# huahbo/IBAMR

Measured on AMD Instinct MI355X. Metric: IB_4 3D spread+interp marker-ops/sec (fp64) + % HBM roofline, 1/2/4/8 GPU, higher is better.
Workload: dtype f64; 1 GPU; cfg4: 1024^3 periodic staggered grid, 1e8 uniform markers (seed 1234), IB_4, z-slabs; kernel=IB_4, markers=100000000, parallelism=z-slab x1, marker_order=cell, layout=packed, spread_mode=one rank, move=False, renumber=False, spread_into=zeroed f (LDataManager::spread, LDataManager.cpp:596), overlap=False

## Files before the change

### ibamr_amd/csrc/le_sweep.hip

```cpp
#include <hip/hip_runtime.h>

#include <climits>
#include <type_traits>
#include <cstdio>
#include <cstdlib>

#include "le_internal.h"
#include "le_stencil.h"

namespace ibtk_le {

constexpr int SW = 64;
#ifndef IBTK_LE_DIAG_SPREAD
#define IBTK_LE_DIAG_SPREAD 0
#endif

__device__ __forceinline__ double lds_ld(const double* q) {
    return *(const volatile __attribute__((address_space(3))) double*)q;
}

__device__ __forceinline__ int lane_id() { return __lane_id(); }

struct D3 {
    double v[3];
// ... 617 lines not shown
        const double Xraw = (FAM == 2) ? p.X[(int64_t)3 * s + d] : Xs[d];
        stencil1d<K>(Xs[d], Xraw, cd.xlo[d], p.bg.dx[d], cd.ilower[d], cd.lo[d], cd.hi[d], d == cd.axis, p.K6, st[d]);
    }
    const int ox = st[0].icl - gx0, oy = st[1].icl - gy0, oz = st[2].icl - zorg;
    bool ok;
    if constexpr (FAM == 0) {
        ok = ox >= 0 && ox + W <= RX - cd.xcell && oy >= 0 && oy + W <= S::RY - cd.ycell && oz >= a + S::LO &&
             oz + W - 1 <= a + S::HI;
    } else {
        bool empty = false;
#pragma unroll
        for (int d = 0; d < 3; ++d) empty = empty || st[d].ist > st[d].isp;
        if (empty) return 0.0;
        ok = ox + st[0].ist >= 0 && ox + st[0].isp < RX && oy + st[1].ist >= 0 && oy + st[1].isp < S::RY &&
             oz + st[2].ist >= a + S::LO && oz + st[2].isp <= a + S::HI;
    }
    if (!ok) {
        atomicOr(p.err, 1);
        return 0.0;
    }
    double acc = 0.0;
    if constexpr (FAM == 3) {
        acc = ring[islot<K>(oz) * PV + oy * RX + ox];
    } else if constexpr (FAM == 0) {
        const double* base = ring + oy * RX + ox;
        constexpr int R = W <= 4 ? W : (W <= 6 ? 3 : 2);
#pragma unroll
        for (int i2 = 0; i2 < W; ++i2) {
            const double* pl = base + islot<K>(oz + i2) * PV;
#pragma unroll
            for (int r0 = 0; r0 < W; r0 += R) {
                double v[R * W];
#pragma unroll
                for (int r = 0; r < R; ++r)
#pragma unroll
                    for (int i0 = 0; i0 < W; ++i0)
                        v[r * W + i0] = lds_ld(&pl[(r0 + r) * RX + i0]);
#pragma unroll
                for (int r = 0; r < R; ++r) {
                    const double wyz = st[1].w[r0 + r] * st[2].w[i2];
#pragma unroll
                    for (int i0 = 0; i0 < W; ++i0) {
                        const double wt = st[0].w[i0] * wyz;
                        acc = acc + wt * v[r * W + i0];
                    }
                }
            }
        }

    } else {
        double w[3][W];
        int o[3][W];
#pragma unroll
        for (int d = 0; d < 3; ++d) {
#pragma unroll
            for (int i = 0; i < W; ++i) {
                const bool in = i >= st[d].ist && i <= st[d].isp;
                w[d][i] = in ? st[d].w[i] : 0.0;
                o[d][i] = min(max(i, st[d].ist), st[d].isp);
            }
        }
#pragma unroll
        for (int i2 = 0; i2 < W; ++i2) {
            const double* pl = ring + islot<K>(oz + o[2][i2]) * PV + oy * RX + ox;
#pragma unroll
            for (int i1 = 0; i1 < W; ++i1) {
#pragma unroll
                for (int i0 = 0; i0 < W; ++i0)
                    acc = acc + w[0][i0] * w[1][i1] * w[2][i2] * pl[o[1][i1] * RX + o[0][i0]];
            }
        }
    }
    return acc;
}

constexpr int LVL_REC = 32;
__device__ __forceinline__ unsigned lvl_class(const int2* tab, int dx, int dy, int dz, int n0, int n1, int n2,
                                              int64_t s1, int64_t s2) {
    const int2 e = tab[dx + 3 * dy + 9 * dz];
    const int64_t shift = e.y ? (int64_t)dx * n0 + (int64_t)dy * n1 * s1 + (int64_t)dz * n2 * s2 : 0;
    return (unsigned)e.x - (unsigned)(8 * shift);
}
template <int K, bool LVL, bool LF = false>
__global__ __launch_bounds__(SW * IWAVES) void k_interp_sweep(Params p) {
    static_assert(LVL || !LF, "the fused fill is a level's");
    using S = ISh<K>;
    constexpr int LO = S::LO, HI = S::HI, RX = S::RX, NPT = S::NPT;
    __shared__ double ring[S::NSL * S::PVP];
    const int it = sweep_item(p, p.ncomp);
    if (it < 0) return;
    int c;
    SweepItem si;
    item_decode(p, it, c, si);
    const int col = si.col;
    const int a0 = si.p0, a1 = si.p1;
    const int lane = lane_id();
    const int w = __builtin_amdgcn_readfirstlane((int)threadIdx.x >> 6);
    ColGeom cg;
    CompDesc cd;
    const int* bs;
    item_patch<LVL>(p, si, c, cg, cd, bs);
    gdouble* const sorted_X = cur_sorted_X(p);
    if (p.zmode) {
        const bool inner = cg.org[2] + a0 + LO >= p.zlo && cg.org[2] + a1 - 1 + HI <= p.zhi;
        if (inner != (p.zmode == 1)) return;
    }
    {
        bool any = false;
        for (int a = a0 + lane; a < a1; a += SW) any = any || bs[bucket(cg, a, col, NBAND)] > bs[bucket(cg, a, col, 0)];
        if (!__any(any)) return;
    }
    const int cx = col % cg.ncx, cy = col / cg.ncx;
    const int gx0 = cg.org[0] + cx * COLX + LO, gy0 = cg.org[1] + cy * COLY + LO;
    const int zorg = cg.org[2];
    const int nlast = p.nsorted - 1;
    auto image = [&](int i, int d) {
        if (!p.iper[d] || (i >= cd.ilower[d] && i <= cd.iupper[d])) return i;
        const int n = cd.iupper[d] - cd.ilower[d] + 1;
        int r = (i - cd.ilower[d]) % n;
        return cd.ilower[d] + (r < 0 ? r + n : r);
    };
    const bool xlast = S::FAM == 0 && cd.xcell, ylast = S::FAM == 0 && cd.ycell;
    unsigned poff[NPT];
#pragma unroll
    for (int k = 0; k < NPT; ++k) {
        const int q = min(lane + SW * k, S::PV - 1);
        const int qx = q % RX, qy = q / RX;
        const int gx = gx0 + qx, gy = gy0 + qy;
        const bool in = gx >= cd.lo[0] && gx <= cd.hi[0] && gy >= cd.lo[1] && gy <= cd.hi[1] &&
                        !(xlast && qx == RX - 1) && !(ylast && qy == S::RY - 1);
        poff[k] = in ? 8u * (unsigned)((image(gx, 0) - cd.lo[0]) + (image(gy, 1) - cd.lo[1]) * (int)cd.s1) : OFF_NONE;
    }
    constexpr bool lfill = LF;
    unsigned lsel = 0;
    struct Cls {
        unsigned o0, o1, o2, o3;
    };
    Cls ob_m{}, ob_0{}, ob_p{};
    const double* lbase = nullptr;
    unsigned lspan = 0;
    int sxd = 0, syd = 0;
    if constexpr (LF) {
        {
            sxd = gx0 < cd.ilower[0] ? -1 : (gx0 + RX - 1 >= cd.ilower[0] + p.lvl_n[0] ? 1 : 0);
            syd = gy0 < cd.ilower[1] ? -1 : (gy0 + S::RY - 1 >= cd.ilower[1] + p.lvl_n[1] ? 1 : 0);
            const int2* rec = p.lvl_nbr + ((int64_t)c * p.npatch + si.patch) * LVL_REC;
            const int2* tab = rec + 13;
            const int n0 = p.lvl_n[0], n1 = p.lvl_n[1], n2 = p.lvl_n[2];
            const int64_t s1 = cd.s1, s2 = cd.s2;
            ob_m = Cls{lvl_class(tab, 0, 0, -1, n0, n1, n2, s1, s2), lvl_class(tab, sxd, 0, -1, n0, n1, n2, s1, s2),
                       lvl_class(tab, 0, syd, -1, n0, n1, n2, s1, s2), lvl_class(tab, sxd, syd, -1, n0, n1, n2, s1, s2)};
            ob_0 = Cls{lvl_class(tab, 0, 0, 0, n0, n1, n2, s1, s2), lvl_class(tab, sxd, 0, 0, n0, n1, n2, s1, s2),
                       lvl_class(tab, 0, syd, 0, n0, n1, n2, s1, s2), lvl_class(tab, sxd, syd, 0, n0, n1, n2, s1, s2)};
            ob_p = Cls{lvl_class(tab, 0, 0, 1, n0, n1, n2, s1, s2), lvl_class(tab, sxd, 0, 1, n0, n1, n2, s1, s2),
                       lvl_class(tab, 0, syd, 1, n0, n1, n2, s1, s2), lvl_class(tab, sxd, syd, 1, n0, n1, n2, s1, s2)};
            const int2 wb = rec[27], ws = rec[28];
            lbase = reinterpret_cast<const double*>(((uint64_t)(unsigned)wb.y << 32) | (unsigned)wb.x);
            lspan = (unsigned)ws.x;
#pragma unroll
            for (int k = 0; k < NPT; ++k) {
                const int q = min(lane + SW * k, S::PV - 1);
                const int gx = gx0 + q % RX, gy = gy0 + q / RX;
                const bool bx = gx < cd.ilower[0] || gx >= cd.ilower[0] + p.lvl_n[0];
                const bool by = gy < cd.ilower[1] || gy >= cd.ilower[1] + p.lvl_n[1];
                lsel |= ((bx ? 1u : 0u) | (by ? 2u : 0u)) << (2 * k);
            }
        }
    }
    const int plast = a1 - 1 + HI;
    const unsigned plane_bytes = (unsigned)(8 * cd.s2);
    auto plane_load = [&](int zr, double* v) __attribute__((always_inline)) {
        const int z0 = zorg + min(zr, plast);
        const bool zin = z0 >= cd.lo[2] && z0 <= cd.hi[2];
        if constexpr (LF) {
            {
                const int dz = z0 < cd.ilower[2] ? -1 : (z0 >= cd.ilower[2] + p.lvl_n[2] ? 1 : 0);
                const unsigned zo = (unsigned)(8 * (int64_t)(z0 - cd.lo[2]) * cd.s2);
                const unsigned mm = 0u - (unsigned)(dz < 0), mp = 0u - (unsigned)(dz > 0), m0 = ~(mm | mp);
                const unsigned O0 = ((ob_m.o0 & mm) | (ob_0.o0 & m0) | (ob_p.o0 & mp)) + zo;
                const unsigned O1 = ((ob_m.o1 & mm) | (ob_0.o1 & m0) | (ob_p.o1 & mp)) + zo;
                const unsigned O2 = ((ob_m.o2 & mm) | (ob_0.o2 & m0) | (ob_p.o2 & mp)) + zo;
                const unsigned O3 = ((ob_m.o3 & mm) | (ob_0.o3 & m0) | (ob_p.o3 & mp)) + zo;
                const auto pb = plane_rsrc(lbase, zin ? lspan : 0u);
#pragma unroll
                for (int k = 0; k < NPT; ++k) {
                    const unsigned cl = (lsel >> (2 * k)) & 3u;
                    const unsigned o = (cl & 2u) ? ((cl & 1u) ? O3 : O2) : ((cl & 1u) ? O1 : O0);
                    v[k] = buf_ld(pb, poff[k] == OFF_NONE ? OFF_NONE : poff[k] + o);
                }
                return;
            }
        }
        const int z = zin ? image(z0, 2) : z0;
        const int zc = min(max(z, cd.lo[2]), cd.hi[2]);
        const auto pb = plane_rsrc(cd.u + (int64_t)(zc - cd.lo[2]) * cd.s2, zin ? plane_bytes : 0u);
#pragma unroll
        for (int k = 0; k < NPT; ++k) v[k] = buf_ld(pb, poff[k]);
    };
    auto plane_put = [&](int zr, const double* v) {
        double* sl = ring + islot<K>(zr) * S::PVP;
#pragma unroll
        for (int k = 0; k < NPT; ++k)
            if (S::PV % SW == 0 || k < NPT - 1 || lane + SW * k < S::PV) sl[lane + SW * k] = v[k];
    };
    struct Mk {
        int s;
        int q;
        double X[3];
    };
    auto lds_barrier = [&]() {
        asm volatile("s_waitcnt lgkmcnt(0)" ::: "memory");
        __builtin_amdgcn_s_barrier();
        asm volatile("" ::: "memory");
    };

    struct GSpan {
        int beg[IWAVES];
        int pre[IWAVES + 1];
    };
    auto gspan_load = [&](int a) {
        const int k = lane < IWAVES ? lane : min(lane - IWAVES, IWAVES - 1);
        const int ac = min(a + k, cg.nz - 1);
        return bs[bucket(cg, ac, col, lane >= IWAVES && lane < 2 * IWAVES ? NBAND : 0)];
    };
    auto gspan_get = [&](int a, int v, GSpan& gsp) {
        int acc = 0;
#pragma unroll
        for (int k = 0; k < IWAVES; ++k) {
            const int b = __builtin_amdgcn_readlane(v, k);
            const int e = a + k < a1 ? __builtin_amdgcn_readlane(v, IWAVES + k) : b;
            gsp.beg[k] = b;
            gsp.pre[k] = acc;
            acc += e - b;
        }
        gsp.pre[IWAVES] = acc;
    };
    auto chunk_load = [&](const GSpan& gsp, int a, int c, Mk& m, int& am) {
        const int tot = gsp.pre[IWAVES];
        const int j = min(SW * c + lane, max(tot - 1, 0));
        int e = gsp.beg[0] + j, k = 0;
#pragma unroll
        for (int q = 1; q < IWAVES; ++q)
            if (j >= gsp.pre[q]) {
                e = gsp.beg[q] + (j - gsp.pre[q]);
                k = q;
            }
        am = a + k;
        e = min(e, nlast);
        m.s = p.sorted_s[e];
        m.q = (p.qdst ? p.qdst : p.sorted_s)[e];
        const D3 xs = ld3(sorted_X + (int64_t)3 * e);
        m.X[0] = xs.v[0];
        m.X[1] = xs.v[1];
        m.X[2] = xs.v[2];
    };
    auto process_pool = [&](int n, const Mk& m, int am) {
        const bool act = lane < n;
        double acc = 0.0;
        if (act) acc = interp_marker<K>(p, cd, ring, gx0, gy0, zorg, am, m.X, m.s);
        double* dst = (act && m.q >= 0) ? p.Qout + ((int64_t)p.Q_depth * m.q + cd.qcomp) : p.sink + lane;
        *dst = acc;
    };
    double pv[NPT];
    for (int z = a0 + LO + w; z < a0 + HI; z += IWAVES) {
        plane_load(z, pv);
        plane_put(z, pv);
    }
    plane_load(a0 + w + HI, pv);
    GSpan gs;
    gspan_get(a0, gspan_load(a0), gs);
    Mk nxt;
    int anx;
    chunk_load(gs, a0, w, nxt, anx);
    int vsp1 = gspan_load(a0 + IWAVES);
    for (int a = a0; a < a1; a += IWAVES) {
        const int my = a + w;
        lds_barrier();
        plane_put(my + HI, pv);
        lds_barrier();
        const Mk cur = nxt;
        const int acur = anx;
        const GSpan gc = gs;

        gspan_get(a + IWAVES, vsp1, gs);
        chunk_load(gs, a + IWAVES, w, nxt, anx);
        vsp1 = gspan_load(a + 2 * IWAVES);
        plane_load(my + IWAVES + HI, pv);
        const int tot = gc.pre[IWAVES];
        if (SW * w < tot) {
            Mk m = cur;
            int am = acur;
            for (int c = w; SW * c < tot; c += IWAVES) {
                const Mk now = m;
                const int anow = am;
                if (SW * (c + IWAVES) < tot) chunk_load(gc, a, c + IWAVES, m, am);
                process_pool(min(tot - SW * c, SW), now, anow);
            }
        }
    }
}

constexpr int I3C = 3;
constexpr int I3PAD = 11;
constexpr int I3WPC = 4, I3PF = 1;
template <int K> struct I3Sh {
    using S = ISh<K>;
    static constexpr int RSTR = S::NSL * S::PVP + I3PAD;
    static constexpr size_t lds = sizeof(double) * I3C * RSTR;
    static constexpr bool fits = S::FAM == 0 && lds <= 160 * 1024;
};
template <int K, int WPC, int PF>
__global__ __launch_bounds__(SW * I3C * WPC) void k_interp3(Params p) {
    using S = ISh<K>;
    static_assert(I3Sh<K>::fits, "k_interp3: closed-form kernels whose three rings fit the LDS");
    static_assert(IWAVES % WPC == 0, "a component's new planes of a group split evenly over its waves");
    constexpr int LO = S::LO, HI = S::HI, RX = S::RX, NPT = S::NPT, PVP = S::PVP;
    constexpr int PPW = IWAVES / WPC;
    constexpr int I3M = WPC * SW;
    constexpr int RSTR = I3Sh<K>::RSTR;
    __shared__ double ring[I3C * RSTR];
    const int it = sweep_item(p, 1);
    if (it < 0) return;
    const SweepItem si = p.items[it];
    const int col = si.col;
    const int a0 = si.p0, a1 = si.p1;
    const int lane = lane_id();
    const int w = __builtin_amdgcn_readfirstlane((int)threadIdx.x >> 6);
    const int cw = w / WPC, jw = w - cw * WPC;
    const ColGeom& cg = p.cg;
    const int* const bs = p.plane_start;
    gdouble* const sorted_X = cur_sorted_X(p);
    if (p.zmode) {
        const bool inner = cg.org[2] + a0 + LO >= p.zlo && cg.org[2] + a1 - 1 + HI <= p.zhi;
        if (inner != (p.zmode == 1)) return;
    }
    {
        bool any = false;
        for (int a = a0 + lane; a < a1; a += SW) any = any || bs[bucket(cg, a, col, NBAND)] > bs[bucket(cg, a, col, 0)];
        if (!__any(any)) return;
    }
    const int cx = col % cg.ncx, cy = col / cg.ncx;
    const int gx0 = cg.org[0] + cx * COLX + LO, gy0 = cg.org[1] + cy * COLY + LO;
    const int zorg = cg.org[2];
    const int nlast = p.nsorted - 1;
    const CompDesc cd = cw == 0 ? p.comp[0] : (cw == 1 ? p.comp[1] : p.comp[2]);
    auto image = [&](int i, int d) {
        if (!p.iper[d] || (i >= cd.ilower[d] && i <= cd.iupper[d])) return i;
        const int n = cd.iupper[d] - cd.ilower[d] + 1;
        int r = (i - cd.ilower[d]) % n;
        return cd.ilower[d] + (r < 0 ? r + n : r);
    };
    const bool xlast = cd.xcell, ylast = cd.ycell;
    unsigned poff[NPT];
#pragma unroll
    for (int k = 0; k < NPT; ++k) {
        const int q = min(lane + SW * k, S::PV - 1);
        const int qx = q % RX, qy = q / RX;
        const int gx = gx0 + qx, gy = gy0 + qy;
        const bool in = gx >= cd.lo[0] && gx <= cd.hi[0] && gy >= cd.lo[1] && gy <= cd.hi[1] &&
                        !(xlast && qx == RX - 1) && !(ylast && qy == S::RY - 1);
        poff[k] = in ? 8u * (unsigned)((image(gx, 0) - cd.lo[0]) + (image(gy, 1) - cd.lo[1]) * (int)cd.s1) : OFF_NONE;
    }
    const int plast = a1 - 1 + HI;
    const unsigned plane_bytes = (unsigned)(8 * cd.s2);
    auto plane_load = [&](int zr, double* v) __attribute__((always_inline)) {
        const int z0 = zorg + min(zr, plast);
        const bool zin = z0 >= cd.lo[2] && z0 <= cd.hi[2];
        const int z = zin ? image(z0, 2) : z0;
        const int zc = min(max(z, cd.lo[2]), cd.hi[2]);
        const auto pb = plane_rsrc(cd.u + (int64_t)(zc - cd.lo[2]) * cd.s2, zin ? plane_bytes : 0u);
#pragma unroll
        for (int k = 0; k < NPT; ++k) v[k] = buf_ld(pb, poff[k]);
    };
    double* const ring_w = ring + cw * RSTR;
    auto plane_put = [&](int zr, const double* v) {
        double* sl = ring_w + islot<K>(zr) * PVP;
#pragma unroll
        for (int k = 0; k < NPT; ++k)
            if (S::PV % SW == 0 || k < NPT - 1 || lane + SW * k < S::PV) sl[lane + SW * k] = v[k];
    };
    const int cl = (int)threadIdx.x % I3C, ml = (int)threadIdx.x / I3C;
    CompDesc cdl;
#define I3SEL(f) cdl.f = cl == 0 ? p.comp[0].f : (cl == 1 ? p.comp[1].f : p.comp[2].f)
#pragma unroll
    for (int d = 0; d < 3; ++d) {
        I3SEL(xlo[d]);
        I3SEL(ilower[d]);
        I3SEL(lo[d]);
        I3SEL(hi[d]);
    }
    I3SEL(axis);
    I3SEL(xcell);
    I3SEL(ycell);
    I3SEL(qcomp);
#undef I3SEL
    const double* const ring_l = ring + cl * RSTR;
    struct Mk {
        int q;
        double X[3];
    };
    auto lds_barrier = [&]() {
        asm volatile("s_waitcnt lgkmcnt(0)" ::: "memory");
        __builtin_amdgcn_s_barrier();
        asm volatile("" ::: "memory");
    };
    struct GSpan {
        int beg[IWAVES];
        int pre[IWAVES + 1];
    };
    auto gspan_load = [&](int a) {
        const int k = lane < IWAVES ? lane : min(lane - IWAVES, IWAVES - 1);
        const int ac = min(a + k, cg.nz - 1);
        return bs[bucket(cg, ac, col, lane >= IWAVES && lane < 2 * IWAVES ? NBAND : 0)];
    };
    auto gspan_get = [&](int a, int v, GSpan& gsp) {
        int acc = 0;
#pragma unroll
        for (int k = 0; k < IWAVES; ++k) {
            const int b = __builtin_amdgcn_readlane(v, k);
            const int e = a + k < a1 ? __builtin_amdgcn_readlane(v, IWAVES + k) : b;
            gsp.beg[k] = b;
            gsp.pre[k] = acc;
            acc += e - b;
        }
        gsp.pre[IWAVES] = acc;
    };
    auto mk_load = [&](const GSpan& gsp, int a, int r, Mk& m, int& am) {
        const int tot = gsp.pre[IWAVES];
        const int j = min(I3M * r + ml, max(tot - 1, 0));
        int e = gsp.beg[0] + j, k = 0;
#pragma unroll
        for (int q = 1; q < IWAVES; ++q)
            if (j >= gsp.pre[q]) {
                e = gsp.beg[q] + (j - gsp.pre[q]);
                k = q;
            }
        am = a + k;
        e = min(e, nlast);
        m.q = (p.qdst ? p.qdst : p.sorted_s)[e];
        const D3 xs = ld3(sorted_X + (int64_t)3 * e);
        m.X[0] = xs.v[0];
        m.X[1] = xs.v[1];
        m.X[2] = xs.v[2];
    };
    auto process = [&](int n, const Mk& m, int am) {
        const bool act = ml < n;
        double acc = 0.0;
        if (act) acc = interp_marker<K>(p, cdl, ring_l, gx0, gy0, zorg, am, m.X, 0);
        double* dst = (act && m.q >= 0) ? p.Qout + ((int64_t)p.Q_depth * m.q + cdl.qcomp) : p.sink + lane;
        *dst = acc;
    };
    {
        double pv[NPT];
        for (int z = a0 + LO + jw; z < a0 + HI; z += WPC) {
            plane_load(z, pv);
            plane_put(z, pv);
        }
    }
    double pv[PF][PPW][NPT];
#pragma unroll
    for (int b = 0; b < PF; ++b)
#pragma unroll
        for (int t = 0; t < PPW; ++t) plane_load(a0 + b * IWAVES + jw + WPC * t + HI, pv[b][t]);
    GSpan gs;
    gspan_get(a0, gspan_load(a0), gs);
    Mk nxt;
    int anx;
    mk_load(gs, a0, 0, nxt, anx);
    int vsp1 = gspan_load(a0 + IWAVES);
    auto group = [&](int a, double (*pvb)[NPT]) __attribute__((always_inline)) {
        lds_barrier();
#pragma unroll
        for (int t = 0; t < PPW; ++t) plane_put(a + jw + WPC * t + HI, pvb[t]);
        lds_barrier();
        const Mk cur = nxt;
        const int acur = anx;
        const GSpan gc = gs;
        gspan_get(a + IWAVES, vsp1, gs);
        mk_load(gs, a + IWAVES, 0, nxt, anx);
        vsp1 = gspan_load(a + 2 * IWAVES);
#pragma unroll
        for (int t = 0; t < PPW; ++t) plane_load(a + PF * IWAVES + jw + WPC * t + HI, pvb[t]);
        const int tot = gc.pre[IWAVES];
        Mk m = cur;
        int am = acur;
        for (int r = 0; I3M * r < tot; ++r) {
            const Mk now = m;
            const int anow = am;
            if (I3M * (r + 1) < tot) mk_load(gc, a, r + 1, m, am);
            process(min(tot - I3M * r, I3M), now, anow);
        }
    };
    for (int a = a0; a < a1; a += PF * IWAVES) {
#pragma unroll
        for (int b = 0; b < PF; ++b)
            if (b == 0 || a + b * IWAVES < a1) group(a + b * IWAVES, pv[b]);
    }
}

__global__ __launch_bounds__(BLOCK) void k_interp_outside_col(Params p, int n) {
    const int first = p.plane_start[p.nbuckets_total];
    for (int e = first + blockIdx.x * BLOCK + threadIdx.x; e < n; e += gridDim.x * BLOCK) {
        const int s = p.qdst ? p.qdst[e] : p.sorted_s[e];
        if (s < 0) continue;
        for (int c = 0; c < p.ncomp; ++c) p.Qout[(int64_t)p.Q_depth * s + p.comp[c].qcomp] = 0.0;
    }
}

template <int K, bool ZC = false> struct SSh {
    using T = KT<K>;
    static constexpr int W = T::W, LO = T::LO, HI = T::HI, FAM = T::FAM;
    static_assert(!ZC || FAM == 0, "the key-frame ring: closed-form kernels");
    static constexpr int HIE = ZC ? HI - 1 : HI;
    static constexpr int NS = HIE - LO + 1;
    static constexpr int NSL = NS + 1;
    static constexpr int PV = COLX * COLY;
    static constexpr int NPL = PV / SW;
    static constexpr int NR = 11;
    static_assert(NS <= 16, "plane field");
    static_assert(COLX == 32 && COLY % 4 == 0 && COLY >= 8, "32-point rows of 4 x 4 tiles; bands need COLY >= 8");
};

__device__ __forceinline__ void ring_xy(int i, int& x, int& y) {
    const int t = i >> 4, j = i & 15;
    x = 4 * (t % (COLX / 4)) + (j & 3);
    y = 4 * (t / (COLX / 4)) + (j >> 2);
}
__device__ __forceinline__ int ring_wrapped(int x, int y) {
    const int xw = x & (COLX - 1);
    const int yw = ((y % COLY) + COLY) % COLY;
    return 16 * ((xw >> 2) + (COLX / 4) * (yw >> 2)) + (xw & 3) + 4 * (yw & 3);
}

template <class S> __device__ __forceinline__ int sslot(int prel) {
    return (int)((unsigned)(prel + 16 * S::NSL) % (unsigned)S::NSL);
}

struct Ranges {
    int start[SSh<K_IB_4>::NR];
    int pre[SSh<K_IB_4>::NR + 1];
};
__device__ __forceinline__ void make_ranges_lanes(const int* rowv, Ranges& R) {
    constexpr int NR = SSh<K_IB_4>::NR;
    constexpr int rr[NR] = {0, 0, 0, 0, 0, 1, 2, 2, 2, 2, 2};
    constexpr int ib[NR] = {8, 11, 14, 17, 20, 6, 6, 9, 12, 15, 18};
    constexpr int ie[NR] = {9, 12, 15, 18, 21, 21, 7, 10, 13, 16, 19};
    int acc = 0;
#pragma unroll
    for (int r = 0; r < NR; ++r) {
        const int b = __builtin_amdgcn_readlane(rowv[rr[r]], ib[r]);
        const int e = __builtin_amdgcn_readlane(rowv[rr[r]], ie[r]);
        R.start[r] = b;
        R.pre[r] = acc;
        acc += e - b;
    }
    R.pre[NR] = acc;
}
__device__ __forceinline__ int range_pos(const Ranges& R, int j) {
    constexpr int NR = SSh<K_IB_4>::NR;
    int pos = R.start[0] + j;
#pragma unroll
    for (int r = 1; r < NR; ++r)
        if (j >= R.pre[r]) pos = R.start[r] + (j - R.pre[r]);
    return pos;
}

constexpr int CS_PTAB = 2048;
__device__ __forceinline__ bool ca_decode(const Params& p, int ca, ColGeom& cg, int& col, int& a, const int*& bs,
                                          int& zb, double& zxlo, int& zilo, const int* ptab) {
    int base = 0;
    if (p.pd) {
        int lo = 0, hi = p.npatch - 1;
        while (lo < hi) {
            const int mid = (lo + hi + 1) >> 1;
            if ((ptab ? ptab[mid] : p.pd[mid].bucket_base / NBAND) <= ca) lo = mid;
            else hi = mid - 1;
        }
        const PatchDesc& P = p.pd[lo];
        cg = P.cg;
        base = P.bucket_base / NBAND;
        bs = p.plane_start + P.bucket_base;
        zb = P.ca_base_z;
        zxlo = P.xlo[2] - 0.5 * p.bg.dx[2];
        zilo = P.ilower[2];
    } else {
        cg = p.cg;
        bs = p.plane_start;
        zb = 0;
        zxlo = p.bg.xlo[2] - 0.5 * p.bg.dx[2];
        zilo = p.bg.ilower[2];
    }
    const int l = ca - base;
    col = l / cg.nz;
    a = l - col * cg.nz;
    zb += col * (cg.nz + 1) + a;
    const int cx = col % cg.ncx, cy = col / cg.ncx;
    return !(cx == 0 || cx == cg.ncx - 1 || cy == 0 || cy == cg.ncy - 1);
}
__device__ __forceinline__ void ca_range(const ColGeom& cg, const int* bs, int col, int a, int r, int& b, int& e) {
    constexpr int rr[11] = {0, 0, 0, 0, 0, 1, 2, 2, 2, 2, 2};
    constexpr int ib[11] = {8, 11, 14, 17, 20, 6, 6, 9, 12, 15, 18};
    constexpr int ie[11] = {9, 12, 15, 18, 21, 21, 7, 10, 13, 16, 19};
    const int cx = col % cg.ncx, cy = col / cg.ncx;
    const int base = bucket(cg, a, (cy - 1 + rr[r]) * cg.ncx + (cx - 1), 0);
    b = bs[base + ib[r]];
    e = bs[base + ie[r]];
}
constexpr int CS_GRID = 8192;
__device__ __forceinline__ bool cs_stands(const Params& p) {
    return p.items_skip && *p.items_skip == 0 && (!p.cs_off_z || *p.cs_zflip != p.cs_epoch);
}
__device__ __forceinline__ const int* cs_patch_table(const Params& p, int* ptab) {
    if (!p.pd || p.npatch > CS_PTAB) return nullptr;
    for (int q = threadIdx.x; q < p.npatch; q += BLOCK) ptab[q] = p.pd[q].bucket_base / NBAND;
    __syncthreads();
    return ptab;
}
__global__ __launch_bounds__(BLOCK) void k_cand_count(Params p, int ncl, int* cnt) {
    if (cs_stands(p)) return;
    __shared__ int ptab_s[CS_PTAB];
    const int* const ptab = cs_patch_table(p, ptab_s);
    for (int ca = blockIdx.x * BLOCK + threadIdx.x; ca < ncl; ca += gridDim.x * BLOCK) {
        ColGeom cg;
        int col, a, zb, zilo;
        double zxlo;
        const int* bs;
        int t = 0;
        if (ca_decode(p, ca, cg, col, a, bs, zb, zxlo, zilo, ptab)) {
#pragma unroll
            for (int r = 0; r < 11; ++r) {
                int b, e;
                ca_range(cg, bs, col, a, r, b, e);
                t += e - b;
            }
        }
        cnt[ca] = t;
    }
}
struct CaJob {
    ColGeom cg;
    int col, a, zb, zilo, o, t;
    double zxlo;
    bool items;
    const int* bs;
    int rowv[3];
    Ranges R;
    int e0;
    double z0;
};
template <bool SHZ>
__global__ __launch_bounds__(BLOCK) void k_cand_write(Params p, int ncl, const int* off, int* pos,
                                                      const unsigned long long* total) {
    if (cs_stands(p)) return;
    if (*total >= (unsigned long long)p.cs_total + 1ull) {
        if (blockIdx.x == 0 && threadIdx.x == 0) atomicOr(p.err, 16);
        return;
    }
    const int lane = threadIdx.x & (SW - 1);
    const int nw = gridDim.x * (BLOCK / SW);
    gdouble* const sX = cur_sorted_X(p);
    const double inv_dz = 1.0 / p.bg.dx[2];
    int* const offz = const_cast<int*>(p.cs_off_z);
    __shared__ int ptab_s[CS_PTAB];
    const int* const ptab = cs_patch_table(p, ptab_s);
    auto load_rows = [&](int ca, CaJob& J) {
        J.items = ca < ncl && ca_decode(p, ca, J.cg, J.col, J.a, J.bs, J.zb, J.zxlo, J.zilo, ptab);
        J.o = off[min(ca, ncl - 1)];
        if (p.pd) J.items = J.items && off[min(ca + 1, ncl)] != J.o;
        if (J.items) {
            const int cx = J.col % J.cg.ncx, cy = J.col / J.cg.ncx;
            const int col0 = (cy - 1) * J.cg.ncx + (cx - 1);
#pragma unroll
            for (int r = 0; r < 3; ++r) J.rowv[r] = J.bs[bucket(J.cg, J.a, col0 + r * J.cg.ncx, 0) + min(lane, 27)];
        }
    };
    auto load_first = [&](CaJob& J) {
        J.t = 0;
        J.e0 = 0;
        J.z0 = 0.0;
        if (!J.items) return;
        make_ranges_lanes(J.rowv, J.R);
        J.t = J.R.pre[SSh<K_IB_4>::NR];
        J.e0 = range_pos(J.R, min(lane, max(J.t - 1, 0)));
        if constexpr (SHZ) J.z0 = sX[(int64_t)3 * min(J.e0, p.nsorted - 1) + 2];
    };
    auto finish = [&](int ca, CaJob& J) {
        if (ca >= ncl) return;
        const int o = J.o;
        if (SHZ && lane == 0) {
            if (J.a == 0) offz[J.zb] = o;
            if (ca == ncl - 1) offz[J.zb + 2] = off[ca + 1];
        }
        const int t = J.t;
        if constexpr (!SHZ) {
            if (lane < t) pos[o + lane] = J.e0;
            for (int j = lane + SW; j < t; j += SW) pos[o + j] = range_pos(J.R, j);
        } else {
            const int aa = J.a + J.cg.org[2] - J.zilo;
            int nlo = 0, nup = 0;
            for (int j0 = 0; j0 < t; j0 += SW) {
                const int j = j0 + lane;
                int e = J.e0;
                double z = J.z0;
                if (j0 > 0) {
                    e = range_pos(J.R, min(j, t - 1));
                    z = sX[(int64_t)3 * e + 2];
                }
                const double xo = (z - J.zxlo) * inv_dz;
                const int n = p.cs_rint ? (int)__builtin_rint(xo) : d_nint(xo);
                const bool in = j < t;
                const bool up = in && n > aa;
                const unsigned long long bu = __ballot(up), bl = __ballot(in && !up);
                const unsigned long long below = (1ull << lane) - 1ull;
                if (in) {
                    if (up) pos[o + t - 1 - (nup + __popcll(bu & below))] = e;
                    else pos[o + nlo + __popcll(bl & below)] = e;
                }
                nlo += __popcll(bl);
                nup += __popcll(bu);
            }
            if (lane == 0) offz[J.zb + 1] = o + nlo;
        }
    };
    for (int ca = blockIdx.x * (BLOCK / SW) + (int)(threadIdx.x / SW); ca < ncl; ca += nw) {
        CaJob J;
        load_rows(ca, J);
        load_first(J);
        finish(ca, J);
    }
}
hipError_t launch_cand_stream(const Params& p, int ncl, int* cnt, int* off, int* pos, void* temp, size_t temp_bytes,
                              unsigned long long* total, hipStream_t s) {
    if (ncl <= 0) return hipSuccess;
    hipLaunchKernelGGL(k_cand_count, dim3(std::min((ncl + BLOCK - 1) / BLOCK, CS_GRID)), dim3(BLOCK), 0, s, p, ncl,
                       cnt);
    hipError_t e = hipMemsetAsync(total, 0, sizeof(unsigned long long), s);
    if (e != hipSuccess) return e;
    if (p.cs_total >= 0x7fffffff && (e = launch_sum64(cnt, ncl, total, s)) != hipSuccess) return e;
    e = launch_scan(temp, temp_bytes, cnt, off, ncl + 1, s);
    if (e != hipSuccess) return e;
    const int per = BLOCK / SW;
    const dim3 g(std::min((ncl + per - 1) / per, CS_GRID)), b(BLOCK);
    if (p.cs_off_z) hipLaunchKernelGGL(k_cand_write<true>, g, b, 0, s, p, ncl, off, pos, total);
    else hipLaunchKernelGGL(k_cand_write<false>, g, b, 0, s, p, ncl, off, pos, total);
    return hipGetLastError();
}

struct Cand {
    double X[3];
    double V;
    int s;
};

template <typename T> __device__ __forceinline__ void rot4(T* w, int r) {
    const bool b0 = r & 1, b1 = r & 2;
    const T c0 = b0 ? w[1] : w[0], c1 = b0 ? w[2] : w[1], c2 = b0 ? w[3] : w[2], c3 = b0 ? w[0] : w[3];
    w[0] = b1 ? c2 : c0;
    w[1] = b1 ? c3 : c1;
    w[2] = b1 ? c0 : c2;
    w[3] = b1 ? c1 : c3;
}

template <int W> struct TileAdds {
    static constexpr int NA = W == 6 ? 40 : W * W;
    double P[NA];
    int off[NA];
    double wz[W];
    int z0, z1;
    int sl;
};
template <int K, bool CNT, bool ZC, typename Before>
__device__ __forceinline__ void spread_setup(const Params& p, const CompDesc& cd, const Cand& cdat, bool act, int a,
                                             int X0, int Y0, int zorg, int xlo, int xhi, int ylo, int yhi, int plo,
                                             int phi, double inv_h3, const double* inv_d, unsigned long long* cnt,
                                             Before&& before, TileAdds<SSh<K, ZC>::W>& T) {
    using S = SSh<K, ZC>;
    constexpr int W = S::W, FAM = S::FAM, NSL = S::NSL;
    constexpr bool ROT = W >= 4;
    St<W> st[3];
#pragma unroll
    for (int d = 0; d < 3; ++d) {
        const double Xraw = (FAM == 2) ? p.X[(int64_t)3 * cdat.s + d] : cdat.X[d];
#if IBTK_LE_DIAG_SPREAD & 2
        {
            const double xo = (cdat.X[d] - cd.xlo[d]) * inv_d[d];
            st[d].icl = (int)__builtin_rint(xo) + cd.ilower[d] - W / 2;
            st[d].ist = 0;
            st[d].isp = W - 1;
#pragma unroll
            for (int i = 0; i < W; ++i) st[d].w[i] = 0.25 + 0.01 * i;
            (void)Xraw;
        }
#else
        if constexpr (K == K_IB_4) {
            const double xo = (cdat.X[d] - cd.xlo[d]) * inv_d[d];
            const double n = __builtin_rint(xo);
            st[d].icl = (int)n + cd.ilower[d] - 2;
            const double r = xo - (n - 0.5);
            const double q = sqrt_1_2(1.0 + 4.0 * r * (1.0 - r));
            const double ta = 3.0 - 2.0 * r, tb = 1.0 + 2.0 * r;
// ... 832 lines not shown
```

Before: 8.420 billion marker-ops/s.

## Move interp3 per-lane offsets and component rows to LDS, deepen plane prefetch

```diff
diff --git a/ibamr_amd/csrc/le_sweep.hip b/ibamr_amd/csrc/le_sweep.hip
--- a/ibamr_amd/csrc/le_sweep.hip
+++ b/ibamr_amd/csrc/le_sweep.hip
@@ -943,12 +943,20 @@
 
 constexpr int I3C = 3;
 constexpr int I3PAD = 11;
-constexpr int I3WPC = 4, I3PF = 1;
+#ifndef IBTK_LE_I3PF
+#define IBTK_LE_I3PF 2
+#endif
+constexpr int I3WPC = 4, I3PF = IBTK_LE_I3PF;
 template <int K> struct I3Sh {
     using S = ISh<K>;
     static constexpr int RSTR = S::NSL * S::PVP + I3PAD;
     static constexpr size_t lds = sizeof(double) * I3C * RSTR;
     static constexpr bool fits = S::FAM == 0 && lds <= 160 * 1024;
+};
+struct I3Row {
+    double xlo[3];
+    int ilower[3], lo[3], hi[3];
+    int axis, xcell, ycell, qcomp;
 };
 template <int K, int WPC, int PF>
 __global__ __launch_bounds__(SW * I3C * WPC) void k_interp3(Params p) {
@@ -960,6 +968,8 @@
     constexpr int I3M = WPC * SW;
     constexpr int RSTR = I3Sh<K>::RSTR;
     __shared__ double ring[I3C * RSTR];
+    __shared__ unsigned pofft[I3C * NPT * SW];
+    __shared__ I3Row crow[I3C];
     const int it = sweep_item(p, 1);
     if (it < 0) return;
     const SweepItem si = p.items[it];
@@ -991,17 +1001,34 @@
         int r = (i - cd.ilower[d]) % n;
         return cd.ilower[d] + (r < 0 ? r + n : r);
     };
-    const bool xlast = cd.xcell, ylast = cd.ycell;
-    unsigned poff[NPT];
-#pragma unroll
-    for (int k = 0; k < NPT; ++k) {
-        const int q = min(lane + SW * k, S::PV - 1);
-        const int qx = q % RX, qy = q / RX;
-        const int gx = gx0 + qx, gy = gy0 + qy;
-        const bool in = gx >= cd.lo[0] && gx <= cd.hi[0] && gy >= cd.lo[1] && gy <= cd.hi[1] &&
-                        !(xlast && qx == RX - 1) && !(ylast && qy == S::RY - 1);
-        poff[k] = in ? 8u * (unsigned)((image(gx, 0) - cd.lo[0]) + (image(gy, 1) - cd.lo[1]) * (int)cd.s1) : OFF_NONE;
-    }
+    if (jw == 0) {
+        const bool xlast = cd.xcell, ylast = cd.ycell;
+#pragma unroll
+        for (int k = 0; k < NPT; ++k) {
+            const int q = min(lane + SW * k, S::PV - 1);
+            const int qx = q % RX, qy = q / RX;
+            const int gx = gx0 + qx, gy = gy0 + qy;
+            const bool in = gx >= cd.lo[0] && gx <= cd.hi[0] && gy >= cd.lo[1] && gy <= cd.hi[1] &&
+                            !(xlast && qx == RX - 1) && !(ylast && qy == S::RY - 1);
+            pofft[(cw * NPT + k) * SW + lane] =
+                in ? 8u * (unsigned)((image(gx, 0) - cd.lo[0]) + (image(gy, 1) - cd.lo[1]) * (int)cd.s1) : OFF_NONE;
+        }
+        if (lane == 0) {
+            I3Row& r = crow[cw];
+#pragma unroll
+            for (int d = 0; d < 3; ++d) {
+                r.xlo[d] = cd.xlo[d];
+                r.ilower[d] = cd.ilower[d];
+                r.lo[d] = cd.lo[d];
+                r.hi[d] = cd.hi[d];
+            }
+            r.axis = cd.axis;
+            r.xcell = cd.xcell;
+            r.ycell = cd.ycell;
+            r.qcomp = cd.qcomp;
+        }
+    }
+    const unsigned* const poff_w = pofft + cw * NPT * SW + lane;
     const int plast = a1 - 1 + HI;
     const unsigned plane_bytes = (unsigned)(8 * cd.s2);
     auto plane_load = [&](int zr, double* v) __attribute__((always_inline)) {
@@ -1011,7 +1038,7 @@
         const int zc = min(max(z, cd.lo[2]), cd.hi[2]);
         const auto pb = plane_rsrc(cd.u + (int64_t)(zc - cd.lo[2]) * cd.s2, zin ? plane_bytes : 0u);
 #pragma unroll
-        for (int k = 0; k < NPT; ++k) v[k] = buf_ld(pb, poff[k]);
+        for (int k = 0; k < NPT; ++k) v[k] = buf_ld(pb, poff_w[SW * k]);
     };
     double* const ring_w = ring + cw * RSTR;
     auto plane_put = [&](int zr, const double* v) {
@@ -1021,20 +1048,6 @@
             if (S::PV % SW == 0 || k < NPT - 1 || lane + SW * k < S::PV) sl[lane + SW * k] = v[k];
     };
     const int cl = (int)threadIdx.x % I3C, ml = (int)threadIdx.x / I3C;
-    CompDesc cdl;
-#define I3SEL(f) cdl.f = cl == 0 ? p.comp[0].f : (cl == 1 ? p.comp[1].f : p.comp[2].f)
-#pragma unroll
-    for (int d = 0; d < 3; ++d) {
-        I3SEL(xlo[d]);
-        I3SEL(ilower[d]);
-        I3SEL(lo[d]);
-        I3SEL(hi[d]);
-    }
-    I3SEL(axis);
-    I3SEL(xcell);
-    I3SEL(ycell);
-    I3SEL(qcomp);
-#undef I3SEL
     const double* const ring_l = ring + cl * RSTR;
     struct Mk {
         int q;
@@ -1087,10 +1100,27 @@
     auto process = [&](int n, const Mk& m, int am) {
         const bool act = ml < n;
         double acc = 0.0;
+        int rl = cl;
+        asm volatile("" : "+v"(rl));
+        const I3Row* rw = crow + rl;
+        CompDesc cdl;
+#pragma unroll
+        for (int d = 0; d < 3; ++d) {
+            cdl.xlo[d] = rw->xlo[d];
+            cdl.ilower[d] = rw->ilower[d];
+            cdl.lo[d] = rw->lo[d];
+            cdl.hi[d] = rw->hi[d];
+        }
+        cdl.axis = rw->axis;
+        cdl.xcell = rw->xcell;
+        cdl.ycell = rw->ycell;
         if (act) acc = interp_marker<K>(p, cdl, ring_l, gx0, gy0, zorg, am, m.X, 0);
-        double* dst = (act && m.q >= 0) ? p.Qout + ((int64_t)p.Q_depth * m.q + cdl.qcomp) : p.sink + lane;
+        double* dst = (act && m.q >= 0) ? p.Qout + ((int64_t)p.Q_depth * m.q + rw->qcomp) : p.sink + lane;
         *dst = acc;
     };
+    lds_barrier();
+    const int vsp0 = gspan_load(a0);
+    int vsp1 = gspan_load(a0 + IWAVES);
     {
         double pv[NPT];
         for (int z = a0 + LO + jw; z < a0 + HI; z += WPC) {
@@ -1098,17 +1128,16 @@
             plane_put(z, pv);
         }
     }
-    double pv[PF][PPW][NPT];
-#pragma unroll
-    for (int b = 0; b < PF; ++b)
-#pragma unroll
-        for (int t = 0; t < PPW; ++t) plane_load(a0 + b * IWAVES + jw + WPC * t + HI, pv[b][t]);
     GSpan gs;
-    gspan_get(a0, gspan_load(a0), gs);
+    gspan_get(a0, vsp0, gs);
     Mk nxt;
     int anx;
     mk_load(gs, a0, 0, nxt, anx);
-    int vsp1 = gspan_load(a0 + IWAVES);
+    double pv[PF][PPW][NPT];
+#pragma unroll
+    for (int b = 0; b < PF; ++b)
+#pragma unroll
+        for (int t = 0; t < PPW; ++t) plane_load(a0 + b * IWAVES + jw + WPC * t + HI, pv[b][t]);
     auto group = [&](int a, double (*pvb)[NPT]) __attribute__((always_inline)) {
         lds_barrier();
 #pragma unroll
@@ -1123,20 +1152,29 @@
 #pragma unroll
         for (int t = 0; t < PPW; ++t) plane_load(a + PF * IWAVES + jw + WPC * t + HI, pvb[t]);
         const int tot = gc.pre[IWAVES];
+        auto mk_wait = [](Mk& k, int& ak) {
+            asm volatile("" : "+v"(k.q), "+v"(k.X[0]), "+v"(k.X[1]), "+v"(k.X[2]), "+v"(ak));
+        };
         Mk m = cur;
         int am = acur;
+        mk_wait(m, am);
+#pragma clang loop unroll(disable)
         for (int r = 0; I3M * r < tot; ++r) {
-            const Mk now = m;
-            const int anow = am;
-            if (I3M * (r + 1) < tot) mk_load(gc, a, r + 1, m, am);
-            process(min(tot - I3M * r, I3M), now, anow);
-        }
-    };
-    for (int a = a0; a < a1; a += PF * IWAVES) {
-#pragma unroll
-        for (int b = 0; b < PF; ++b)
-            if (b == 0 || a + b * IWAVES < a1) group(a + b * IWAVES, pv[b]);
-    }
+            if (r > 0) {
+                mk_load(gc, a, r, m, am);
+                mk_wait(m, am);
+            }
+            process(min(tot - I3M * r, I3M), m, am);
+        }
+    };
+    int a = a0;
+    for (; a + (PF - 1) * IWAVES < a1; a += PF * IWAVES) {
+#pragma unroll
+        for (int b = 0; b < PF; ++b) group(a + b * IWAVES, pv[b]);
+    }
+#pragma unroll
+    for (int b = 0; b < PF - 1; ++b)
+        if (a + b * IWAVES < a1) group(a + b * IWAVES, pv[b]);
 }
 
 __global__ __launch_bounds__(BLOCK) void k_interp_outside_col(Params p, int n) {
```

Result: no change. 8.418 billion marker-ops/s (-0.0%).
